# LukasHaas/PIGEON

Measured on AMD Instinct MI355X. Metric: images/sec end-to-end (ViT+head+refine), 4x336x336, higher is better.
Workload: dtype f16

## Files before the change

### include/pigeon_hip.h

```cpp
#ifndef PIGEON_HIP_H
#define PIGEON_HIP_H

#include <stddef.h>
#include <stdint.h>

#ifdef __cplusplus
extern "C" {
#endif

#define PG_OK            0
#define PG_EINVAL       -1
#define PG_ENOMEM       -2
#define PG_EHIP         -3
#define PG_ESTATE       -4

#define PG_DTYPE_F32     0
#define PG_DTYPE_BF16    1
#define PG_DTYPE_F16     2
#define PG_DTYPE_F64     3

#define PG_ABI_VERSION   7

const char* pg_last_error(void);
int pg_abi_version(void);
int pg_device_count(void);

typedef struct pg_vit pg_vit;

typedef struct pg_vit_cfg {
    int32_t layers;
    int32_t image_size;
    int32_t patch;
    int32_t hidden;
    int32_t heads;
    int32_t mlp;
    float   ln_eps;
    int32_t max_chunk;
    int32_t mma_dtype;
    int32_t precise;
} pg_vit_cfg;

int pg_vit_create(pg_vit** out, int device, const pg_vit_cfg* cfg);
int pg_vit_load_weight(pg_vit* h, const char* name, const void* data, int dtype,
                       const int64_t* shape, int ndim);
int pg_vit_finalize(pg_vit* h);
int pg_vit_workspace_bytes(const pg_vit* h, int n_images, size_t* bytes);
int pg_vit_forward(pg_vit* h, const void* pixels, int pix_dtype, int n_images, float* emb_out,
                   void* workspace, size_t workspace_bytes, void* stream);
int pg_vit_forward_hidden(pg_vit* h, const void* pixels, int pix_dtype, int n_images, float* emb_out,
                          float* hidden_out, void* workspace, size_t workspace_bytes, void* stream);
int pg_vit_precise_workspace_bytes(const pg_vit* h, int n_images, size_t* bytes);
int pg_vit_precise_plan(int n_images, int32_t out[8]);
int pg_vit_forward_precise(pg_vit* h, const void* pixels, int pix_dtype, int n_images, float* emb_out, float* hidden_out,
                           void* workspace, size_t workspace_bytes, void* stream);
int pg_vit_graph(pg_vit* h, int on, int64_t* replays, int64_t* captures);
int pg_vit_destroy(pg_vit* h);
int pg_vit_mma_dtype(const pg_vit* h);

int pg_fingerprint(const void* data, size_t bytes, uint64_t seed, uint64_t out[2], void* stream);
int pg_vit_fingerprint(const pg_vit* h, uint64_t out[2]);

#define PG_PROF_CLASSES 9
int pg_vit_profile_enable(pg_vit* h, int on);
int pg_vit_profile_read(pg_vit* h, int64_t* launches , double* ms );
int pg_vit_profile_reset(pg_vit* h);

int pg_tune_gemm_stagger(float fraction);
int pg_tune_gemm_tail_rows(int rows);
int pg_tune_gemm_tail_shape(int min_k, int min_n);
int pg_tune_gemm_raster(int gn);
int pg_tune_gemm_mid(int on);
int pg_gemm_plan(int variant, int epi, int M, int N, int K, int* kernel, int* rows_main, int* rest);
int pg_tune_exact_attention(int use_f32_mfma);
int pg_tune_exact_products(int n);
int pg_tune_exact_fusion(int on);
int pg_vit_saturation_check(pg_vit* h, int on);
int pg_vit_saturation_read(pg_vit* h, int64_t* count, int reset);
int pg_vit_range_alarm_read(pg_vit* h, int64_t* rows, int reset);

int pg_head_forward(const float* emb, int B, int P, const float* W, const float* bias,
                    const double* centroids, int C, int k, float* logits,
                    float* topk_val, int64_t* topk_idx, int64_t* argmax, double* pred_llh, void* stream);

int pg_head_margin(const float* logits, int B, int C, const float* emb, int P, const float* W, float* margin, float* sens,
                   int64_t* top2, void* stream);

int pg_head_certainty(const float* logits, int B, int C, const float* emb, int P, const float* W, const int64_t* topk_idx, int kx,
                      const float* beta, const float* wstats, float* tol, int32_t* code, float* margin, float* sens, void* stream);

int pg_aux_heads_forward(const float* emb, int B, int P, const float* W, const float* bias, int n_reg, int n_climate, int n_month,
                         const float* beta, float* preds, int64_t* cls, float* tol, int32_t* code, float* row_tol, void* stream);

typedef struct pg_bank {
    const float*   proto_emb;
    const int64_t* cell_off;
    const float*   proto_lnglat;
    const int32_t* proto_count;
    const int64_t* member_off;
    const int64_t* member_idx;
    const float*   train_emb;
    const float*   train_lnglat;
    int64_t num_cells;
    int64_t num_protos;
    int64_t num_train;
} pg_bank;

int pg_refine_forward(const pg_bank* bank, const float* q, int B, int P, const double* init_llh,
                      const int64_t* cand, const float* cand_prob, int k, int topk,
                      float temperature, double max_refine_km, float* scratch,
                      float* out_llh, int64_t* out_cell, int32_t* out_choice, void* stream);

int pg_refine_forward_ex(const pg_bank* bank, const float* q, int B, int P, const double* init_llh,
                         const int64_t* cand, const float* cand_prob, int k, int topk, int n_eval,
                         float temperature, double max_refine_km, float* scratch12,
                         float* out_llh, int64_t* out_cell, int32_t* out_choice, int32_t* out_refined, void* stream);

int pg_refine_certainty(const pg_bank* bank, const float* q, int B, int P, const int64_t* cand, const float* cand_prob, int k,
                        int topk, int n_eval, const float* scratch12, const float* W, int C, const float* beta,
                        const float* wstats, float temperature, const int32_t* refined, const int32_t* choice,
                        float* tol, int32_t* code, void* stream);

int pg_requeue_append(const float* head_tol, const float* refine_tol, const int32_t* refine_code, int B, float thr, int force_all,
                      int64_t dst_base, int64_t flushed, int64_t cap, int64_t* counters, int64_t* slot_dst, int32_t* row_slot,
                      uint8_t* certain, int32_t* cause, void* stream);
int pg_rows_to_slots(const void* src, int64_t row_bytes, const int32_t* row_slot, int B, void* dst, void* stream);
int pg_requeue_take(const int64_t* slot_dst, int64_t cap, int64_t head, int n_valid, int n_pad, int64_t* dst_out, void* stream);
int pg_scatter_rows(const void* src, int64_t row_bytes, const int64_t* dst_row, int n, void* dst, int64_t dst_rows,
                    int64_t remap_wb, int64_t remap_b, int64_t remap_off, void* stream);
int pg_head_wstats(const float* W, int C, const float* beta, float* out2, void* stream);

int pg_embedding_debias(float* emb, int64_t n, int dim, const float* bias, void* stream);

typedef struct pg_prep pg_prep;
int pg_prep_create(pg_prep** out, int device, int in_h, int in_w);
int pg_prep_destroy(pg_prep* h);
int pg_prep_geometry(const pg_prep* h, int32_t* out6);
int pg_prep_workspace_bytes(const pg_prep* h, int n_images, size_t* bytes);
int pg_prep_forward(pg_prep* h, const void* images_u8, int n_images, void* out, int out_dtype, void* workspace,
                    size_t workspace_bytes, void* stream);

#define PG_PREP_ITEM_BYTES 80
#define PG_PREP_RAGGED_MAX_IMAGES 65535
typedef struct pg_prep_item {
    uint64_t src_off;
    int32_t in_h, in_w;
    int32_t new_h, new_w, top, left;
    int32_t ksize_h, ksize_v;
    int32_t row0, nrows;
    int32_t tmp_row;
    uint32_t bounds_h_off, kk_h_off, bounds_v_off, kk_v_off;
    int32_t reserved[3];
} pg_prep_item;
int pg_prep_ragged_plan(int n, const int32_t* hw, pg_prep_item* items_out, size_t* packed_bytes, size_t* workspace_bytes);
typedef struct pg_prep_ragged pg_prep_ragged;
int pg_prep_ragged_create(pg_prep_ragged** out, int device);
int pg_prep_ragged_destroy(pg_prep_ragged* h);
int pg_prep_ragged_forward(pg_prep_ragged* h, const void* packed_dev, size_t packed_bytes, const pg_prep_item* items_host, int n,
                           void* out, int out_dtype, void* workspace, size_t workspace_bytes, void* stream);

#define PG_COMM_ID_BYTES 128
int pg_comm_unique_id(void* id_out );
int pg_comm_init_rank(void** comm, int nranks, const void* unique_id , int rank);
int pg_comm_count(void* comm, int* nranks);
int pg_allgather(void* comm, const void* send, void* recv, size_t bytes_per_rank, void* stream);
int pg_allgather_many(void* comm, int count, const void* const* send, void* const* recv, const size_t* bytes_per_rank,
                      void* stream);
int pg_comm_destroy(void* comm);
int pg_comm_rccl_version(void);

int pg_proto_build(const float* train_emb, int panels, int64_t num_train, const int64_t* member_off,
                   const int64_t* member_idx, int64_t num_protos, float* proto_emb, void* stream);
int pg_haversine_matrix(const void* x, int x_dtype, const double* y, int N, int M, double* out, void* stream);
int pg_haversine_pairs(const double* x, const void* y, int y_dtype, int64_t N, double* out, void* stream);
int pg_smooth_labels(const double* distances, int N, int M, double constant, double* out, void* stream);

int pg_haversine_blocks(const double* pts, const int64_t* cell_off, const int64_t* mat_off, int C, double zero_as, double* out,
                        void* stream);
int pg_optics_graph(const double* dist, const int64_t* cell_off, const int64_t* mat_off, int C, int min_samples, int64_t* ordering,
                    double* core, double* reach, int64_t* pred, void* stream);
int pg_optics_plan(int64_t n, int min_samples, int32_t out[4]);
int pg_tune_optics_lds_points(int max_points);

int pg_op_gemm16(int dtype, const void* A, int64_t lda, const void* W, const float* bias, void* out, int64_t ldc,
                 int M, int N, int K, int epi, float qscale, int qcols, const float* aux,
                 int variant, void* stream);
int pg_op_gemm16_ld(int dtype, const void* A, int64_t lda, const void* W, int64_t ldw, const float* bias, void* out,
                    int64_t ldc, int M, int N, int K, int epi, float qscale, int qcols, const float* aux,
                    int variant, void* stream);
int pg_op_rowstat_cast(const float* x, void* x16, int dtype, float* rowstat, int64_t rows, float eps, void* stream);
int pg_op_gemm16_resid_stat(int dtype, const void* A, int64_t lda, const void* W, int64_t ldw, const float* bias, float* X,
                            int64_t ldc, void* x16, int64_t ldx, float* statpart, int M, int N, int K, int variant, void* stream);
int pg_op_rowstat_finalize(const float* statpart, int slots, float* rowstat, int64_t rows, float eps, void* stream);
int pg_op_gemm16_ln(int dtype, const void* A, int64_t lda, const void* W, int64_t ldw, const float* bias, const float* colsum,
                    const float* rowstat, void* out, int64_t ldc, int M, int N, int K, int epi, float qscale, int qcols,
                    int variant, void* stream);
int pg_op_layernorm(const float* x, const float* gamma, const float* beta, void* y, int out_dtype,
                    int64_t rows, float eps, void* stream);
int pg_op_attention(int dtype, const void* qkv, void* out, int n_images, void* stream);
int pg_op_im2col(const void* pixels, int pix_dtype, void* out, int out_dtype, int n_images, void* stream);
int pg_op_token_mean(const float* x, float* out, int n_images, void* stream);
int pg_op_cast_f32(const float* x, void* y, int out_dtype, int64_t n, void* stream);
int pg_op_preln(float* x, const float* cls, const float* pos0, const float* gamma, const float* beta, int64_t rows, float eps,
                void* x16, int x16_dtype, float* rowstat, void* stream);
int pg_op_gemm16_parts(int dtype, const void* A, int64_t lda, const void* W, int64_t ldw, const float* bias, float* parts,
                       int M, int N, int Kp, int S, void* stream);
int pg_op_x3_split(const float* x, void* y3, int64_t rows, int cols, int gelu, void* stream);
int pg_op_x3_layernorm(const float* x, const float* gamma, const float* beta, void* y3, int64_t rows, float eps, void* stream);
int pg_op_attention_f32(const float* qkv, float* out, int n_images, void* stream);
int pg_op_attention_x3(const float* qkv, void* out3, int n_images, void* stream);
int pg_op_x3_im2col(const void* pixels, int pix_dtype, void* out3, int n_images, void* stream);
int pg_op_sum_parts(const float* parts, int S, int64_t part_elems, float* dst, int64_t n, int resid, void* stream);

#ifdef __cplusplus
}
#endif
#endif
```

### pigeon_amd/_lib.py

```python
from __future__ import annotations

import ctypes as C
import os

_HERE = os.path.dirname(os.path.abspath(__file__))
LIB_PATH = os.environ.get("PIGEON_HIP_LIB") or os.path.join(_HERE, "libpigeon_hip.so")

PG_DTYPE_F32, PG_DTYPE_BF16, PG_DTYPE_F16, PG_DTYPE_F64 = 0, 1, 2, 3
EPI_QKV, EPI_GELU, EPI_RESID, EPI_PATCH, EPI_F32, EPI_RESID_STAT, EPI_QKV_LN, EPI_GELU_LN, EPI_GELU_X3 = 0, 1, 2, 3, 4, 5, 6, 7, 8
PROF_CLASSES = ["gemm_qkv", "gemm_out", "gemm_fc1", "gemm_fc2", "gemm_patch", "attention", "layernorm",
                "im2col", "token_mean"]


class PigeonHipError(RuntimeError):
    pass


class VitCfg(C.Structure):
    _fields_ = [("layers", C.c_int32), ("image_size", C.c_int32), ("patch", C.c_int32), ("hidden", C.c_int32),
                ("heads", C.c_int32), ("mlp", C.c_int32), ("ln_eps", C.c_float), ("max_chunk", C.c_int32),
                ("mma_dtype", C.c_int32), ("precise", C.c_int32)]


class Bank(C.Structure):
    _fields_ = [("proto_emb", C.c_void_p), ("cell_off", C.c_void_p), ("proto_lnglat", C.c_void_p),
                ("proto_count", C.c_void_p), ("member_off", C.c_void_p), ("member_idx", C.c_void_p),
                ("train_emb", C.c_void_p), ("train_lnglat", C.c_void_p),
                ("num_cells", C.c_int64), ("num_protos", C.c_int64), ("num_train", C.c_int64)]


class PrepItem(C.Structure):
    _fields_ = [("src_off", C.c_uint64), ("in_h", C.c_int32), ("in_w", C.c_int32), ("new_h", C.c_int32), ("new_w", C.c_int32),
                ("top", C.c_int32), ("left", C.c_int32), ("ksize_h", C.c_int32), ("ksize_v", C.c_int32), ("row0", C.c_int32),
                ("nrows", C.c_int32), ("tmp_row", C.c_int32), ("bounds_h_off", C.c_uint32), ("kk_h_off", C.c_uint32),
                ("bounds_v_off", C.c_uint32), ("kk_v_off", C.c_uint32), ("reserved", C.c_int32 * 3)]


PREP_ITEM_BYTES = 80
assert C.sizeof(PrepItem) == PREP_ITEM_BYTES


_P, _I, _I64, _F, _D, _SZ = C.c_void_p, C.c_int, C.c_int64, C.c_float, C.c_double, C.c_size_t
SIGNATURES = {
    "pg_last_error": (C.c_char_p, []),
    "pg_abi_version": (_I, []),
    "pg_device_count": (_I, []),
    "pg_vit_create": (_I, [C.POINTER(_P), _I, C.POINTER(VitCfg)]),
    "pg_vit_load_weight": (_I, [_P, C.c_char_p, _P, _I, C.POINTER(_I64), _I]),
    "pg_vit_finalize": (_I, [_P]),
    "pg_vit_workspace_bytes": (_I, [_P, _I, C.POINTER(_SZ)]),
    "pg_vit_forward": (_I, [_P, _P, _I, _I, _P, _P, _SZ, _P]),
    "pg_vit_forward_hidden": (_I, [_P, _P, _I, _I, _P, _P, _P, _SZ, _P]),
    "pg_vit_precise_workspace_bytes": (_I, [_P, _I, C.POINTER(_SZ)]),
    "pg_vit_forward_precise": (_I, [_P, _P, _I, _I, _P, _P, _P, _SZ, _P]),
    "pg_vit_graph": (_I, [_P, _I, C.POINTER(_I64), C.POINTER(_I64)]),
    "pg_vit_destroy": (_I, [_P]),
    "pg_vit_mma_dtype": (_I, [_P]),
    "pg_fingerprint": (_I, [_P, _SZ, C.c_uint64, C.POINTER(C.c_uint64), _P]),
    "pg_vit_fingerprint": (_I, [_P, C.POINTER(C.c_uint64)]),
    "pg_vit_profile_enable": (_I, [_P, _I]),
    "pg_vit_profile_read": (_I, [_P, C.POINTER(_I64), C.POINTER(_D)]),
    "pg_vit_profile_reset": (_I, [_P]),
    "pg_tune_gemm_stagger": (_I, [_F]),
    "pg_tune_gemm_tail_rows": (_I, [_I]),
    "pg_tune_gemm_tail_shape": (_I, [_I, _I]),
    "pg_tune_gemm_raster": (_I, [_I]),
    "pg_tune_gemm_mid": (_I, [_I]),
    "pg_tune_exact_attention": (_I, [_I]),
    "pg_tune_exact_products": (_I, [_I]),
    "pg_tune_exact_fusion": (_I, [_I]),
    "pg_gemm_plan": (_I, [_I, _I, _I, _I, _I, _P, _P, _P]),
    "pg_vit_saturation_check": (_I, [_P, _I]),
    "pg_vit_saturation_read": (_I, [_P, C.POINTER(_I64), _I]),
    "pg_vit_range_alarm_read": (_I, [_P, C.POINTER(_I64), _I]),
    "pg_comm_unique_id": (_I, [_P]),
    "pg_comm_init_rank": (_I, [C.POINTER(_P), _I, _P, _I]),
    "pg_comm_count": (_I, [_P, C.POINTER(_I)]),
    "pg_allgather": (_I, [_P, _P, _P, _SZ, _P]),
    "pg_allgather_many": (_I, [_P, _I, C.POINTER(_P), C.POINTER(_P), C.POINTER(_SZ), _P]),
    "pg_comm_destroy": (_I, [_P]),
    "pg_comm_rccl_version": (_I, []),
    "pg_prep_create": (_I, [C.POINTER(_P), _I, _I, _I]),
    "pg_prep_destroy": (_I, [_P]),
    "pg_prep_geometry": (_I, [_P, C.POINTER(C.c_int32)]),
    "pg_prep_workspace_bytes": (_I, [_P, _I, C.POINTER(_SZ)]),
    "pg_prep_forward": (_I, [_P, _P, _I, _P, _I, _P, _SZ, _P]),
    "pg_prep_ragged_plan": (_I, [_I, C.POINTER(C.c_int32), C.POINTER(PrepItem), C.POINTER(_SZ), C.POINTER(_SZ)]),
    "pg_prep_ragged_create": (_I, [C.POINTER(_P), _I]),
    "pg_prep_ragged_destroy": (_I, [_P]),
    "pg_prep_ragged_forward": (_I, [_P, _P, _SZ, C.POINTER(PrepItem), _I, _P, _I, _P, _SZ, _P]),
    "pg_proto_build": (_I, [_P, _I, _I64, _P, _P, _I64, _P, _P]),
    "pg_haversine_matrix": (_I, [_P, _I, _P, _I, _I, _P, _P]),
    "pg_haversine_pairs": (_I, [_P, _P, _I, _I64, _P, _P]),
    "pg_smooth_labels": (_I, [_P, _I, _I, _D, _P, _P]),
    "pg_haversine_blocks": (_I, [_P, _P, _P, _I, _D, _P, _P]),
    "pg_optics_graph": (_I, [_P, _P, _P, _I, _I, _P, _P, _P, _P, _P]),
    "pg_optics_plan": (_I, [_I64, _I, C.POINTER(C.c_int32)]),
    "pg_tune_optics_lds_points": (_I, [_I]),
    "pg_head_forward": (_I, [_P, _I, _I, _P, _P, _P, _I, _I, _P, _P, _P, _P, _P, _P]),
    "pg_head_margin": (_I, [_P, _I, _I, _P, _I, _P, _P, _P, _P, _P]),
    "pg_head_certainty": (_I, [_P, _I, _I, _P, _I, _P, _P, _I, _P, _P, _P, _P, _P, _P, _P]),
    "pg_aux_heads_forward": (_I, [_P, _I, _I, _P, _P, _I, _I, _I, _P, _P, _P, _P, _P, _P, _P]),
    "pg_refine_forward": (_I, [C.POINTER(Bank), _P, _I, _I, _P, _P, _P, _I, _I, _F, _D, _P, _P, _P, _P, _P]),
    "pg_refine_forward_ex": (_I, [C.POINTER(Bank), _P, _I, _I, _P, _P, _P, _I, _I, _I, _F, _D, _P, _P, _P, _P, _P, _P]),
    "pg_refine_certainty": (_I, [C.POINTER(Bank), _P, _I, _I, _P, _P, _I, _I, _I, _P, _P, _I, _P, _P, _F, _P, _P, _P, _P, _P]),
    "pg_requeue_append": (_I, [_P, _P, _P, _I, _F, _I, _I64, _I64, _I64, _P, _P, _P, _P, _P, _P]),
    "pg_rows_to_slots": (_I, [_P, _I64, _P, _I, _P, _P]),
    "pg_requeue_take": (_I, [_P, _I64, _I64, _I, _I, _P, _P]),
    "pg_scatter_rows": (_I, [_P, _I64, _P, _I, _P, _I64, _I64, _I64, _I64, _P]),
    "pg_head_wstats": (_I, [_P, _I, _P, _P, _P]),
    "pg_embedding_debias": (_I, [_P, _I64, _I, _P, _P]),
    "pg_op_gemm16": (_I, [_I, _P, _I64, _P, _P, _P, _I64, _I, _I, _I, _I, _F, _I, _P, _I, _P]),
    "pg_op_gemm16_ld": (_I, [_I, _P, _I64, _P, _I64, _P, _P, _I64, _I, _I, _I, _I, _F, _I, _P, _I, _P]),
    "pg_op_rowstat_cast": (_I, [_P, _P, _I, _P, _I64, _F, _P]),
    "pg_op_gemm16_resid_stat": (_I, [_I, _P, _I64, _P, _I64, _P, _P, _I64, _P, _I64, _P, _I, _I, _I, _I, _P]),
    "pg_op_rowstat_finalize": (_I, [_P, _I, _P, _I64, _F, _P]),
    "pg_op_gemm16_ln": (_I, [_I, _P, _I64, _P, _I64, _P, _P, _P, _P, _I64, _I, _I, _I, _I, _F, _I, _I, _P]),
    "pg_op_layernorm": (_I, [_P, _P, _P, _P, _I, _I64, _F, _P]),
    "pg_op_attention": (_I, [_I, _P, _P, _I, _P]),
    "pg_op_im2col": (_I, [_P, _I, _P, _I, _I, _P]),
    "pg_op_token_mean": (_I, [_P, _P, _I, _P]),
    "pg_op_cast_f32": (_I, [_P, _P, _I, _I64, _P]),
    "pg_op_gemm16_parts": (_I, [_I, _P, _I64, _P, _I64, _P, _P, _I, _I, _I, _I, _P]),
    "pg_op_x3_split": (_I, [_P, _P, _I64, _I, _I, _P]),
    "pg_op_x3_layernorm": (_I, [_P, _P, _P, _P, _I64, _F, _P]),
    "pg_op_attention_f32": (_I, [_P, _P, _I, _P]),
    "pg_op_attention_x3": (_I, [_P, _P, _I, _P]),
    "pg_op_x3_im2col": (_I, [_P, _I, _P, _I, _P]),
    "pg_op_sum_parts": (_I, [_P, _I, _I64, _P, _I64, _I, _P]),
    "pg_op_preln": (_I, [_P, _P, _P, _P, _P, _I64, _F, _P, _I, _P, _P]),
    "pg_vit_precise_plan": (_I, [_I, C.POINTER(C.c_int32)]),
}

_lib = None


def load():
    global _lib
    if _lib is not None:
        return _lib
    if not os.path.exists(LIB_PATH):
        raise PigeonHipError(
            f"{LIB_PATH} not found: build it with `python -m pigeon_amd.build` (hipcc, gfx950). "
            "pigeon_amd has no CPU/PyTorch fallback for its hot path.")
    import torch
    lib = C.CDLL(LIB_PATH)
    for name, (res, args) in SIGNATURES.items():
        fn = getattr(lib, name)
        fn.restype = res
        fn.argtypes = args
    _lib = lib
    return lib


def check(rc: int, what: str = ""):
    if rc != 0:
        msg = load().pg_last_error()
        raise PigeonHipError(f"{what} failed (code {rc}): {msg.decode() if msg else ''}")


def require_gpu():
    lib = load()
    n = lib.pg_device_count()
    if n <= 0:
        raise PigeonHipError("pigeon_amd needs an AMD GPU (gfx950) visible to HIP; found none. "
                             "There is no CPU fallback for the hot path.")
    return n
```

### pigeon_amd/csrc/head.hip

```cpp
#include "common.h"
#include "pigeon_internal.h"
#include "certainty_common.h"
#include <cfloat>

#define HT 64
#define HK 32

__global__ __launch_bounds__(256) void head_logits_kernel(const float* __restrict__ emb, int B, int P,
                                                          const float* __restrict__ W, const float* __restrict__ bias,
                                                          int C, float* __restrict__ logits) {
    __shared__ float As[HK][HT + 1];
    __shared__ float Ws[HK][HT + 1];
    const int tid = threadIdx.x;
    const int c0 = blockIdx.x * HT, b0 = blockIdx.y * HT;
    const int tx = tid & 15, ty = tid >> 4;
    float acc[4][4];
#pragma unroll
    for (int i = 0; i < 4; ++i)
#pragma unroll
        for (int j = 0; j < 4; ++j) acc[i][j] = 0.f;
    const float invP = 1.0f / (float)P;
    for (int k0 = 0; k0 < VIT_HIDDEN; k0 += HK) {
#pragma unroll
        for (int i = 0; i < 8; ++i) {
            const int idx = tid + i * 256;
            const int r = idx >> 5, k = idx & 31;
            float a = 0.f;
            if (b0 + r < B) {
                const float* e = emb + ((int64_t)(b0 + r) * P) * VIT_HIDDEN + k0 + k;
                for (int p = 0; p < P; ++p) a += e[(int64_t)p * VIT_HIDDEN];
                a *= invP;
            }
            As[k][r] = a;
            Ws[k][r] = (c0 + r < C) ? W[(int64_t)(c0 + r) * VIT_HIDDEN + k0 + k] : 0.f;
        }
        __syncthreads();
#pragma unroll
        for (int k = 0; k < HK; ++k) {
            float a[4], w[4];
#pragma unroll
            for (int i = 0; i < 4; ++i) a[i] = As[k][ty * 4 + i];
#pragma unroll
            for (int j = 0; j < 4; ++j) w[j] = Ws[k][tx * 4 + j];
#pragma unroll
            for (int i = 0; i < 4; ++i)
#pragma unroll
                for (int j = 0; j < 4; ++j) acc[i][j] = fmaf(a[i], w[j], acc[i][j]);
        }
        __syncthreads();
    }
#pragma unroll
    for (int i = 0; i < 4; ++i) {
        const int b = b0 + ty * 4 + i;
        if (b >= B) continue;
#pragma unroll
        for (int j = 0; j < 4; ++j) {
            const int c = c0 + tx * 4 + j;
            if (c < C) logits[(int64_t)b * C + c] = acc[i][j] + bias[c];
        }
    }
}

struct ValIdx { float v; int i; };
__device__ __forceinline__ ValIdx block_argbest(ValIdx x, ValIdx* red ) {
#pragma unroll
    for (int o = 32; o >= 1; o >>= 1) {
        const float ov = __shfl_xor(x.v, o, 64);
        const int oi = __shfl_xor(x.i, o, 64);
        if (better(ov, oi, x.v, x.i)) { x.v = ov; x.i = oi; }
    }
    const int wave = threadIdx.x >> 6;
    __syncthreads();
    if ((threadIdx.x & 63) == 0) red[wave] = x;
    __syncthreads();
    ValIdx r = red[0];
#pragma unroll
    for (int w = 1; w < 4; ++w) if (better(red[w].v, red[w].i, r.v, r.i)) r = red[w];
    return r;
}

template <bool GLOBAL>
__global__ __launch_bounds__(256) void head_row_kernel(const float* __restrict__ logits, int C, int k,
                                                       const double* __restrict__ centroids,
                                                       float* __restrict__ topk_val, int64_t* __restrict__ topk_idx,
                                                       int64_t* __restrict__ argmax_out, double* __restrict__ pred_llh,
                                                       float* __restrict__ scratch) {
    extern __shared__ __attribute__((aligned(16))) float probs_lds[];
    float* probs = GLOBAL ? scratch + (int64_t)blockIdx.x * C : probs_lds;
    __shared__ ValIdx red[4];
    __shared__ float redf[4];
    const int b = blockIdx.x, tid = threadIdx.x;
    const float* row = logits + (int64_t)b * C;
    float mx = -FLT_MAX;
    for (int c = tid; c < C; c += 256) { const float v = row[c]; probs[c] = v; mx = fmaxf(mx, v); }
    mx = wave_max(mx);
    if ((tid & 63) == 0) redf[tid >> 6] = mx;
    __syncthreads();
    mx = fmaxf(fmaxf(redf[0], redf[1]), fmaxf(redf[2], redf[3]));
    __syncthreads();
    float sm = 0.f;
    for (int c = tid; c < C; c += 256) { const float e = expf(probs[c] - mx); probs[c] = e; sm += e; }
    sm = wave_sum(sm);
    if ((tid & 63) == 0) redf[tid >> 6] = sm;
    __syncthreads();
    sm = (redf[0] + redf[1]) + (redf[2] + redf[3]);
    for (int c = tid; c < C; c += 256) probs[c] = probs[c] / sm;
    __syncthreads();
    for (int r = 0; r < k; ++r) {
        ValIdx best; best.v = -1.f; best.i = 0x7fffffff;
        for (int c = tid; c < C; c += 256) {
            const float v = probs[c];
            if (better(v, c, best.v, best.i)) { best.v = v; best.i = c; }
        }
        best = block_argbest(best, red);
        if (tid == 0) {
            if (best.i < 0 || best.i >= C) best.i = r < C ? r : C - 1;
            topk_val[(int64_t)b * k + r] = best.v;
            topk_idx[(int64_t)b * k + r] = best.i;
            if (r == 0) {
                argmax_out[b] = best.i;
                pred_llh[2 * b] = centroids[2 * (int64_t)best.i];
                pred_llh[2 * b + 1] = centroids[2 * (int64_t)best.i + 1];
            }
            probs[best.i] = -2.f;
        }
        if (GLOBAL) __threadfence_block();
        __syncthreads();
    }
}

extern "C" int pg_head_forward(const float* emb, int B, int P, const float* W, const float* bias,
                               const double* centroids, int C, int k, float* logits, float* topk_val,
                               int64_t* topk_idx, int64_t* argmax, double* pred_llh, void* stream) {
    hipStream_t s = (hipStream_t)stream;
    if (B < 0) { pg_set_error("head: B = %d", B); return PG_EINVAL; }
    if (B == 0) return PG_OK;
    if (!emb || !W || !bias || !centroids || !logits || !topk_val || !topk_idx || !argmax || !pred_llh) {
        pg_set_error("head: null pointer argument"); return PG_EINVAL;
    }
    if (P < 1 || C < 1 || k < 1 || k > C) { pg_set_error("head: bad P=%d C=%d k=%d", P, C, k); return PG_EINVAL; }
    const size_t lds = (size_t)C * sizeof(float);
    const bool big = lds > 150 * 1024;
    dim3 g1((C + HT - 1) / HT, (B + HT - 1) / HT);
    hipLaunchKernelGGL(head_logits_kernel, g1, dim3(256), 0, s, emb, B, P, W, bias, C, logits);
    int rc = pg_check_launch("head_logits");
    if (rc) return rc;
    if (big) {
        float* scratch = nullptr;
        PG_HIP(hipMallocAsync((void**)&scratch, (size_t)B * C * sizeof(float), s));
        hipLaunchKernelGGL(head_row_kernel<true>, dim3(B), dim3(256), 0, s, logits, C, k, centroids, topk_val, topk_idx, argmax, pred_llh, scratch);
        rc = pg_check_launch("head_row (large C)");
        (void)hipFreeAsync(scratch, s);
        return rc;
    }
    static size_t attr_lds = 0;
    if (lds > attr_lds) {
        PG_HIP(hipFuncSetAttribute((const void*)head_row_kernel<false>, hipFuncAttributeMaxDynamicSharedMemorySize, (int)lds));
        attr_lds = lds;
    }
    hipLaunchKernelGGL(head_row_kernel<false>, dim3(B), dim3(256), lds, s, logits, C, k, centroids, topk_val, topk_idx, argmax, pred_llh,
                       (float*)nullptr);
    return pg_check_launch("head_row");
}

__global__ __launch_bounds__(256) void head_margin_kernel(const float* __restrict__ logits, int C, const float* __restrict__ emb, int P,
                                                          const float* __restrict__ W, float* __restrict__ margin,
                                                          float* __restrict__ sens, int64_t* __restrict__ top2) {
    __shared__ ValIdx red[4];
    __shared__ float redf[8];
    const int b = blockIdx.x, tid = threadIdx.x;
    const float* row = logits + (int64_t)b * C;
    ValIdx b1; b1.v = -FLT_MAX; b1.i = 0x7fffffff;
    bool any = false;
    for (int c = tid; c < C; c += 256) { const float v = row[c]; if (!any || better(v, c, b1.v, b1.i)) { b1.v = v; b1.i = c; any = true; } }
    if (!any) { b1.v = -FLT_MAX; b1.i = 0x7fffffff; }
    const ValIdx t1 = block_argbest(b1, red);
    ValIdx b2; b2.v = -FLT_MAX; b2.i = 0x7fffffff;
    any = false;
    for (int c = tid; c < C; c += 256) {
        if (c == t1.i) continue;
        const float v = row[c];
        if (!any || better(v, c, b2.v, b2.i)) { b2.v = v; b2.i = c; any = true; }
    }
    if (!any) { b2.v = -FLT_MAX; b2.i = 0x7fffffff; }
    __syncthreads();
    const ValIdx t2 = block_argbest(b2, red);
    const bool have2 = C > 1 && t2.i >= 0 && t2.i < C;
    float se = 0.f, sw = 0.f;
    {
        const int c0 = tid * 4;
        const float invP = 1.0f / (float)P;
#pragma unroll
        for (int e = 0; e < 4; ++e) {
            float a = 0.f;
            for (int p = 0; p < P; ++p) a += emb[((int64_t)b * P + p) * VIT_HIDDEN + c0 + e];
            a *= invP;
            se += a * a;
            if (have2) { const float d = W[(int64_t)t1.i * VIT_HIDDEN + c0 + e] - W[(int64_t)t2.i * VIT_HIDDEN + c0 + e]; sw += d * d; }
        }
    }
    se = wave_sum(se); sw = wave_sum(sw);
    __syncthreads();
    if ((tid & 63) == 0) { redf[tid >> 6] = se; redf[4 + (tid >> 6)] = sw; }
    __syncthreads();
    if (tid == 0) {
        se = (redf[0] + redf[1]) + (redf[2] + redf[3]);
        sw = (redf[4] + redf[5]) + (redf[6] + redf[7]);
        margin[b] = have2 ? t1.v - t2.v : INFINITY;
        sens[b] = have2 ? sqrtf(se) * sqrtf(sw) * (1.0f / 32.0f) : 0.f;
        if (top2) top2[b] = have2 ? t2.i : t1.i;
    }
}

extern "C" int pg_head_margin(const float* logits, int B, int C, const float* emb, int P, const float* W, float* margin, float* sens,
                              int64_t* top2, void* stream) {
    if (B < 0) { pg_set_error("head_margin: B = %d", B); return PG_EINVAL; }
    if (B == 0) return PG_OK;
    if (!logits || !emb || !W || !margin || !sens) { pg_set_error("head_margin: null pointer argument"); return PG_EINVAL; }
    if (P < 1 || C < 1) { pg_set_error("head_margin: bad P=%d C=%d", P, C); return PG_EINVAL; }
    hipLaunchKernelGGL(head_margin_kernel, dim3(B), dim3(256), 0, (hipStream_t)stream, logits, C, emb, P, W, margin, sens, top2);
    return pg_check_launch("head_margin");
}
```

### pigeon_amd/hip_ops.py

```python
from __future__ import annotations

import ctypes as C
from typing import Dict, Optional

import torch

from . import _lib
from ._lib import Bank, VitCfg, check, load

TOKENS, HIDDEN, MLP, PATCHES, KPAD = 577, 1024, 4096, 576, 640


def _p(t: Optional[torch.Tensor]):
    return C.c_void_p(0) if t is None else C.c_void_p(t.data_ptr())


def _stream():
    return C.c_void_p(torch.cuda.current_stream().cuda_stream)


_T16 = {torch.float16: _lib.PG_DTYPE_F16, torch.bfloat16: _lib.PG_DTYPE_BF16}
_PIXDT = {torch.float32: _lib.PG_DTYPE_F32, torch.float16: _lib.PG_DTYPE_F16, torch.bfloat16: _lib.PG_DTYPE_BF16}
_PG2T = {_lib.PG_DTYPE_F16: torch.float16, _lib.PG_DTYPE_BF16: torch.bfloat16, _lib.PG_DTYPE_F32: torch.float32}

# ... 671 lines not shown
    y = torch.empty((rows, 3 * cols), dtype=torch.float16, device=x.device)
    check(load().pg_op_x3_split(_p(x), _p(y), rows, cols, 1 if gelu else 0, _stream()), "pg_op_x3_split")
    return y


def gemm16_parts(A: torch.Tensor, W: torch.Tensor, bias: Optional[torch.Tensor], S: int) -> torch.Tensor:
    _dev(A); _dev(W)
    if W.dtype != A.dtype or A.shape[1] != W.shape[1] or A.shape[1] % S:
        raise _lib.PigeonHipError("gemm16_parts: A and W must share dtype and a K' divisible by S")
    M, Kt = A.shape
    N = W.shape[0]
    out = torch.empty((S, M, N), dtype=torch.float32, device=A.device)
    check(load().pg_op_gemm16_parts(_dt16(A), _p(A), A.stride(0), _p(W), W.stride(0), _p(bias), _p(out), M, N, Kt // S, S, _stream()),
          "pg_op_gemm16_parts")
    return out


def x3_layernorm(x: torch.Tensor, gamma: torch.Tensor, beta: torch.Tensor, eps: float = 1e-5) -> torch.Tensor:
    _dev(x, torch.float32)
    rows = x.numel() // HIDDEN
    y = torch.empty((rows, 3 * HIDDEN), dtype=torch.float16, device=x.device)
    check(load().pg_op_x3_layernorm(_p(x), _p(gamma), _p(beta), _p(y), rows, float(eps), _stream()), "pg_op_x3_layernorm")
    return y


def x3_pack_weight(W: torch.Tensor) -> torch.Tensor:
    Wh = W.to(torch.float16)
    Wl = ((W - Wh.float()) * 256.0).to(torch.float16)
    return torch.cat([Wh, Wh, Wl], dim=1).contiguous()


def attention_f32(qkv: torch.Tensor, n_images: int) -> torch.Tensor:
    _dev(qkv, torch.float32)
    _shape(qkv, "qkv", n_images * TOKENS, 3 * HIDDEN)
    out = torch.empty((n_images * TOKENS, HIDDEN), dtype=torch.float32, device=qkv.device)
    check(load().pg_op_attention_f32(_p(qkv), _p(out), n_images, _stream()), "pg_op_attention_f32")
    return out


class DeviceBank:

    FIELDS = [("proto_emb", torch.float32), ("cell_off", torch.int64), ("proto_lnglat", torch.float32),
              ("proto_count", torch.int32), ("member_off", torch.int64), ("member_idx", torch.int64),
              ("train_emb", torch.float32), ("train_lnglat", torch.float32)]

    def __init__(self, arrays, device="cuda"):
        self.t = {}
        for name, dt in self.FIELDS:
            a = getattr(arrays, name) if not isinstance(arrays, dict) else arrays[name]
            t = torch.as_tensor(a) if not torch.is_tensor(a) else a
            self.t[name] = t.to(device=device, dtype=dt).contiguous()
        self.num_cells = self.t["cell_off"].numel() - 1
        self.num_protos = self.t["proto_emb"].shape[0]
        self.num_train = self.t["train_emb"].shape[0]
        t = self.t
        _shape(t["proto_emb"], "proto_emb", self.num_protos, HIDDEN); _shape(t["proto_lnglat"], "proto_lnglat", self.num_protos, 2)
        _shape(t["proto_count"], "proto_count", self.num_protos); _shape(t["member_off"], "member_off", self.num_protos + 1)
        _shape(t["cell_off"], "cell_off", self.num_cells + 1); _shape(t["member_idx"], "member_idx", None)
        _shape(t["train_emb"], "train_emb", self.num_train, HIDDEN); _shape(t["train_lnglat"], "train_lnglat", self.num_train, 2)
        self.struct = Bank(*[C.c_void_p(self.t[n].data_ptr()) for n, _ in self.FIELDS],
                           self.num_cells, self.num_protos, self.num_train)


def refine_forward(bank: DeviceBank, q: torch.Tensor, init_llh: torch.Tensor, cand: torch.Tensor,
                   cand_prob: Optional[torch.Tensor], topk: int, temperature: float, max_refine_km: float,
                   return_scratch: bool = False):
    _dev(q, torch.float32); _dev(init_llh, torch.float64); _dev(cand, torch.int64)
    if cand_prob is not None:
        _dev(cand_prob, torch.float32)
    if q.dim() not in (2, 3) or cand.dim() != 2:
        raise _lib.PigeonHipError(f"refine: q must be (B,{HIDDEN}) or (B,P,{HIDDEN}) and cand (B,k), got {tuple(q.shape)} / {tuple(cand.shape)}")
    B = q.shape[0]
    P = q.shape[1] if q.dim() == 3 else 1
    k = cand.shape[1]
    _shape(q, "q", *((B, P, HIDDEN) if q.dim() == 3 else (B, HIDDEN)))
    _shape(init_llh, "init_llh", B, 2); _shape(cand, "cand", B, k)
    if cand_prob is not None:
        _shape(cand_prob, "cand_prob", B, k)
    if not 1 <= int(topk) <= k:
        raise _lib.PigeonHipError(f"refine: topk = {topk} of k = {k} candidates")
    dev = q.device
    scratch = torch.empty((B, topk, 4), dtype=torch.float32, device=dev)
    out_llh = torch.empty((B, 2), dtype=torch.float32, device=dev)
    out_cell = torch.empty((B,), dtype=torch.int64, device=dev)
    out_choice = torch.empty((B,), dtype=torch.int32, device=dev)
    check(load().pg_refine_forward(C.byref(bank.struct), _p(q), B, P, _p(init_llh), _p(cand), _p(cand_prob), k, topk,
                                   float(temperature), float(max_refine_km), _p(scratch), _p(out_llh), _p(out_cell),
                                   _p(out_choice), _stream()), "pg_refine_forward")
    if return_scratch:
        return out_llh, out_cell, out_choice, scratch
    return out_llh, out_cell, out_choice


def refine_forward_ex(bank: DeviceBank, q: torch.Tensor, init_llh: torch.Tensor, cand: torch.Tensor,
                      cand_prob: Optional[torch.Tensor], topk: int, n_eval: int, temperature: float, max_refine_km: float):
    _dev(q, torch.float32); _dev(init_llh, torch.float64); _dev(cand, torch.int64)
    if cand_prob is not None:
        _dev(cand_prob, torch.float32)
    if q.dim() not in (2, 3) or cand.dim() != 2:
        raise _lib.PigeonHipError(f"refine: q must be (B,{HIDDEN}) or (B,P,{HIDDEN}) and cand (B,k), got {tuple(q.shape)} / {tuple(cand.shape)}")
    B = q.shape[0]
    P = q.shape[1] if q.dim() == 3 else 1
    k = cand.shape[1]
    _shape(q, "q", *((B, P, HIDDEN) if q.dim() == 3 else (B, HIDDEN)))
    _shape(init_llh, "init_llh", B, 2); _shape(cand, "cand", B, k)
    if cand_prob is not None:
        _shape(cand_prob, "cand_prob", B, k)
    if not 1 <= int(topk) <= int(n_eval) <= k:
        raise _lib.PigeonHipError(f"refine_ex: topk = {topk}, n_eval = {n_eval} of k = {k} candidates")
    dev = q.device
    scratch = torch.empty((B, n_eval, 12), dtype=torch.float32, device=dev)
    out_llh = torch.empty((B, 2), dtype=torch.float32, device=dev)
    out_cell = torch.empty((B,), dtype=torch.int64, device=dev)
    out_choice = torch.empty((B,), dtype=torch.int32, device=dev)
    out_refined = torch.empty((B,), dtype=torch.int32, device=dev)
    check(load().pg_refine_forward_ex(C.byref(bank.struct), _p(q), B, P, _p(init_llh), _p(cand), _p(cand_prob), k, int(topk), int(n_eval),
                                      float(temperature), float(max_refine_km), _p(scratch), _p(out_llh), _p(out_cell),
                                      _p(out_choice), _p(out_refined), _stream()), "pg_refine_forward_ex")
    return out_llh, out_cell, out_choice, out_refined, scratch


def refine_certainty(bank: DeviceBank, q: torch.Tensor, cand: torch.Tensor, cand_prob: Optional[torch.Tensor], topk: int,
                     scratch12: torch.Tensor, W: torch.Tensor, drift: Optional[torch.Tensor], wstats: torch.Tensor,
                     temperature: float, refined: torch.Tensor, choice: torch.Tensor):
    _dev(q, torch.float32); _dev(cand, torch.int64); _dev(scratch12, torch.float32); _dev(W, torch.float32)
    _dev(wstats, torch.float32); _dev(refined, torch.int32); _dev(choice, torch.int32)
    B = q.shape[0]
    P = q.shape[1] if q.dim() == 3 else 1
    k = cand.shape[1]
    n_eval = scratch12.shape[1]
    _shape(q, "q", *((B, P, HIDDEN) if q.dim() == 3 else (B, HIDDEN)))
    _shape(cand, "cand", B, k); _shape(scratch12, "scratch12", B, n_eval, 12); _shape(W, "W", None, HIDDEN)
    _shape(refined, "refined", B); _shape(choice, "choice", B); _shape(wstats, "wstats", 2)
    if cand_prob is not None:
        _dev(cand_prob, torch.float32); _shape(cand_prob, "cand_prob", B, k)
    if drift is not None:
        _dev(drift, torch.float32); _shape(drift, "drift", HIDDEN)
    tol = torch.empty((B,), dtype=torch.float32, device=q.device)
    code = torch.empty((B,), dtype=torch.int32, device=q.device)
    check(load().pg_refine_certainty(C.byref(bank.struct), _p(q), B, P, _p(cand), _p(cand_prob), k, int(topk), int(n_eval), _p(scratch12),
                                     _p(W), W.shape[0], _p(drift), _p(wstats), float(temperature), _p(refined), _p(choice), _p(tol),
                                     _p(code), _stream()), "pg_refine_certainty")
    return tol, code


def tune_gemm_raster(gn: int) -> None:
    check(load().pg_tune_gemm_raster(int(gn)), "pg_tune_gemm_raster")


def tune_exact_fusion(on: bool) -> None:
    check(load().pg_tune_exact_fusion(1 if on else 0), "pg_tune_exact_fusion")


def tune_gemm_mid(on) -> None:
    mode = 2 if (not isinstance(on, bool) and on == 2) else (1 if on else 0)
    check(load().pg_tune_gemm_mid(mode), "pg_tune_gemm_mid")


def vit_precise_plan(n_images: int) -> dict:
    out = (C.c_int32 * 8)()
    check(load().pg_vit_precise_plan(int(n_images), out), "pg_vit_precise_plan")
    return dict(qkv=out[0], out=out[1], fc1=out[2], fc2=out[3], fc1_fused=bool(out[4]), attn_x3=bool(out[5]), chunk=out[6], chunks=out[7])


def tune_exact_products(n: int) -> None:
    check(load().pg_tune_exact_products(int(n)), "pg_tune_exact_products")


def x3_im2col(pixels: torch.Tensor, out: Optional[torch.Tensor] = None) -> torch.Tensor:
    _dev(pixels); _shape(pixels, "pixels", None, 3, 336, 336)
    n = pixels.shape[0]
    if out is None:
        out = torch.empty((n * PATCHES, 3 * KPAD), dtype=torch.float16, device=pixels.device)
    _dev(out, torch.float16)
    if out.numel() < n * PATCHES * 3 * KPAD:
        raise _lib.PigeonHipError("x3_im2col: output too small")
    check(load().pg_op_x3_im2col(_p(pixels), _PIXDT[pixels.dtype], _p(out), n, _stream()), "pg_op_x3_im2col")
    return out


def sum_parts(parts: torch.Tensor, dst: torch.Tensor, resid: bool, n: Optional[int] = None) -> torch.Tensor:
    _dev(parts, torch.float32); _dev(dst, torch.float32)
    S, pe = parts.shape[0], parts[0].numel()
    n = pe if n is None else int(n)
    if dst.numel() < n:
        raise _lib.PigeonHipError("sum_parts: dst too small")
    check(load().pg_op_sum_parts(_p(parts), S, pe, _p(dst), n, 1 if resid else 0, _stream()), "pg_op_sum_parts")
    return dst


def preln(x: torch.Tensor, cls: torch.Tensor, pos0: torch.Tensor, gamma: torch.Tensor, beta: torch.Tensor, rows: Optional[int] = None,
          eps: float = 1e-5, stat_dtype: Optional[torch.dtype] = None, x16: Optional[torch.Tensor] = None,
          rowstat: Optional[torch.Tensor] = None):
    _dev(x, torch.float32)
    for t in (cls, pos0, gamma, beta):
        _dev(t, torch.float32)
        if t.numel() < HIDDEN:
            raise _lib.PigeonHipError("preln: parameter vectors need 1024 elements")
    rows = x.numel() // HIDDEN if rows is None else int(rows)
    if x.numel() < rows * HIDDEN:
        raise _lib.PigeonHipError("preln: x too small")
    if stat_dtype is not None and x16 is None:
        x16 = torch.empty((rows, HIDDEN), dtype=stat_dtype, device=x.device)
        rowstat = torch.empty((rows, 2), dtype=torch.float32, device=x.device)
    if x16 is not None and (x16.numel() < rows * HIDDEN or rowstat.numel() < rows * 2):
        raise _lib.PigeonHipError("preln: x16 / rowstat too small")
    check(load().pg_op_preln(_p(x), _p(cls), _p(pos0), _p(gamma), _p(beta), rows, float(eps), _p(x16),
                             _dt16(x16) if x16 is not None else 0, _p(rowstat), _stream()), "pg_op_preln")
    return (x16, rowstat) if x16 is not None else None


def attention_x3(qkv: torch.Tensor, n_images: int, out: Optional[torch.Tensor] = None) -> torch.Tensor:
    _dev(qkv, torch.float32)
    _shape(qkv, "qkv", n_images * TOKENS, 3 * HIDDEN)
    if out is None:
        out = torch.empty((n_images * TOKENS, 3 * HIDDEN), dtype=torch.float16, device=qkv.device)
    _dev(out, torch.float16)
    if out.numel() < n_images * TOKENS * 3 * HIDDEN:
        raise _lib.PigeonHipError("attention_x3: output too small")
    check(load().pg_op_attention_x3(_p(qkv), _p(out), n_images, _stream()), "pg_op_attention_x3")
    return out
```

Measured before the change: 2463.

## Stream head weights through double-buffered LDS with DPP broadcast FMAs after separate mean

Replaces the head logits kernel with a two-step path. The patch mean is computed first into a scratch buffer, then a weight-streaming GEMV-style kernel runs. It double-buffers W column tiles through LDS, prefetches the next stage while computing, and uses inline-asm DPP row broadcast FMAs so each lane owns one class column and keeps small batches in registers. The goal is to make the head bandwidth-bound on W rather than recomputing the mean per tile, at the cost of an extra allocation and launch, and of fragile hand-written asm.

```diff
diff --git a/include/pigeon_hip.h b/include/pigeon_hip.h
--- a/include/pigeon_hip.h
+++ b/include/pigeon_hip.h
@@ -78,6 +78,7 @@
 int pg_vit_saturation_read(pg_vit* h, int64_t* count, int reset);
 int pg_vit_range_alarm_read(pg_vit* h, int64_t* rows, int reset);
 
+int pg_tune_head_stream(int on);
 int pg_head_forward(const float* emb, int B, int P, const float* W, const float* bias,
                     const double* centroids, int C, int k, float* logits,
                     float* topk_val, int64_t* topk_idx, int64_t* argmax, double* pred_llh, void* stream);
diff --git a/pigeon_amd/_lib.py b/pigeon_amd/_lib.py
--- a/pigeon_amd/_lib.py
+++ b/pigeon_amd/_lib.py
@@ -97,6 +97,7 @@
     "pg_optics_graph": (_I, [_P, _P, _P, _I, _I, _P, _P, _P, _P, _P]),
     "pg_optics_plan": (_I, [_I64, _I, C.POINTER(C.c_int32)]),
     "pg_tune_optics_lds_points": (_I, [_I]),
+    "pg_tune_head_stream": (_I, [_I]),
     "pg_head_forward": (_I, [_P, _I, _I, _P, _P, _P, _I, _I, _P, _P, _P, _P, _P, _P]),
     "pg_head_margin": (_I, [_P, _I, _I, _P, _I, _P, _P, _P, _P, _P]),
     "pg_head_certainty": (_I, [_P, _I, _I, _P, _I, _P, _P, _I, _P, _P, _P, _P, _P, _P, _P]),
diff --git a/pigeon_amd/csrc/head.hip b/pigeon_amd/csrc/head.hip
--- a/pigeon_amd/csrc/head.hip
+++ b/pigeon_amd/csrc/head.hip
@@ -59,6 +59,217 @@
             if (c < C) logits[(int64_t)b * C + c] = acc[i][j] + bias[c];
         }
     }
+}
+
+#define HS_CT 64
+
+__global__ __launch_bounds__(256) void head_panel_mean_kernel(const float* __restrict__ emb, int B, int P, float* __restrict__ mean) {
+    const int64_t i = (int64_t)blockIdx.x * 256 + threadIdx.x;
+    if (i >= (int64_t)B * VIT_HIDDEN) return;
+    const int64_t b = i / VIT_HIDDEN;
+    const int k = (int)(i % VIT_HIDDEN);
+    const float* e = emb + (b * P) * VIT_HIDDEN + k;
+    float a = 0.f;
+    for (int p = 0; p < P; ++p) a += e[(int64_t)p * VIT_HIDDEN];
+    a *= 1.0f / (float)P;
+    mean[i] = a;
+}
+
+#define HS_FM4(J, WOP)                                                                   \
+    "v_fmac_f32_dpp %0, %4, %" WOP " row_newbcast:" J " row_mask:0xf bank_mask:0xf\n\t"    \
+    "v_fmac_f32_dpp %1, %5, %" WOP " row_newbcast:" J " row_mask:0xf bank_mask:0xf\n\t"    \
+    "v_fmac_f32_dpp %2, %6, %" WOP " row_newbcast:" J " row_mask:0xf bank_mask:0xf\n\t"    \
+    "v_fmac_f32_dpp %3, %7, %" WOP " row_newbcast:" J " row_mask:0xf bank_mask:0xf\n\t"
+#define HS_FM2(J, WOP)                                                                   \
+    "v_fmac_f32_dpp %0, %2, %" WOP " row_newbcast:" J " row_mask:0xf bank_mask:0xf\n\t"    \
+    "v_fmac_f32_dpp %1, %3, %" WOP " row_newbcast:" J " row_mask:0xf bank_mask:0xf\n\t"
+#define HS_W16(w) "v"(w[0]), "v"(w[1]), "v"(w[2]), "v"(w[3]), "v"(w[4]), "v"(w[5]), "v"(w[6]), "v"(w[7]), \
+                  "v"(w[8]), "v"(w[9]), "v"(w[10]), "v"(w[11]), "v"(w[12]), "v"(w[13]), "v"(w[14]), "v"(w[15])
+
+__device__ __forceinline__ void hs_fma16x4(float* acc, const float* a, const float (&w)[16]) {
+    asm("s_nop 4\n\t"
+        HS_FM4("0", "8") HS_FM4("1", "9") HS_FM4("2", "10") HS_FM4("3", "11")
+        HS_FM4("4", "12") HS_FM4("5", "13") HS_FM4("6", "14") HS_FM4("7", "15")
+        HS_FM4("8", "16") HS_FM4("9", "17") HS_FM4("10", "18") HS_FM4("11", "19")
+        HS_FM4("12", "20") HS_FM4("13", "21") HS_FM4("14", "22") HS_FM4("15", "23")
+        : "+v"(acc[0]), "+v"(acc[1]), "+v"(acc[2]), "+v"(acc[3])
+        : "v"(a[0]), "v"(a[1]), "v"(a[2]), "v"(a[3]), HS_W16(w));
+}
+__device__ __forceinline__ void hs_fma16x2(float* acc, const float* a, const float (&w)[16]) {
+    asm("s_nop 4\n\t"
+        HS_FM2("0", "4") HS_FM2("1", "5") HS_FM2("2", "6") HS_FM2("3", "7")
+        HS_FM2("4", "8") HS_FM2("5", "9") HS_FM2("6", "10") HS_FM2("7", "11")
+        HS_FM2("8", "12") HS_FM2("9", "13") HS_FM2("10", "14") HS_FM2("11", "15")
+        HS_FM2("12", "16") HS_FM2("13", "17") HS_FM2("14", "18") HS_FM2("15", "19")
+        : "+v"(acc[0]), "+v"(acc[1])
+        : "v"(a[0]), "v"(a[1]), HS_W16(w));
+}
+
+template <int KC, int NB>
+__device__ __forceinline__ void hs_stage(float (&acc)[NB], const float (&a)[KC / 16][NB], const float* cur, const int lane) {
+    static_assert(NB == 2 || NB % 4 == 0, "rows per wave");
+#pragma unroll
+    for (int sub = 0; sub < KC / 16; ++sub) {
+        float w[16];
+#pragma unroll
+        for (int q = 0; q < 4; ++q) {
+            const float4 v = *reinterpret_cast<const float4*>(&cur[lane * (KC + 4) + sub * 16 + q * 4]);
+            w[q * 4] = v.x; w[q * 4 + 1] = v.y; w[q * 4 + 2] = v.z; w[q * 4 + 3] = v.w;
+        }
+        if constexpr (NB == 2) {
+            hs_fma16x2(&acc[0], &a[sub][0], w);
+        } else {
+#pragma unroll
+            for (int r0 = 0; r0 < NB; r0 += 4) hs_fma16x4(&acc[r0], &a[sub][r0], w);
+        }
+    }
+}
+
+template <int KC, int NB>
+__global__ __launch_bounds__(256, KC == 64 ? 3 : 2) void head_logits_stream_kernel(const float* __restrict__ mean, int B,
+                                                                                   const float* __restrict__ W,
+                                                                                   const float* __restrict__ bias, int C,
+                                                                                   float* __restrict__ logits, int row_blocks) {
+    constexpr int LD = KC + 4;
+    constexpr int NS = VIT_HIDDEN / KC;
+    constexpr int TPR = KC / 4;
+    constexpr int RPP = 256 / TPR;
+    constexpr int NLD = HS_CT / RPP;
+    constexpr int NSUB = KC / 16;
+    static_assert(NS % 2 == 0 && NS >= 4, "the stage loop is unrolled by two");
+    extern __shared__ __attribute__((aligned(16))) float hs_w[];
+    const int tid = threadIdx.x, lane = tid & 63, wave = tid >> 6;
+    int tile = blockIdx.x, rblk = 0;
+    if (row_blocks > 1) {
+        const int slot = blockIdx.x >> 3;
+        tile = (slot / row_blocks) * 8 + (blockIdx.x & 7);
+        rblk = slot % row_blocks;
+    }
+    const int c0 = tile * HS_CT;
+    if (c0 >= C) return;
+    const int b0 = (rblk * 4 + wave) * NB;
+
+    const int scol = (tid % TPR) * 4, srow = tid / TPR;
+    const char* wbase = reinterpret_cast<const char*>(W + (int64_t)c0 * VIT_HIDDEN);
+    const int clast = C - 1 - c0;
+    unsigned woff[NLD];
+#pragma unroll
+    for (int i = 0; i < NLD; ++i) {
+        int c = srow + i * RPP;
+        c = c < clast ? c : clast;
+        woff[i] = (unsigned)(c * VIT_HIDDEN + scol) * 4u;
+    }
+    const int bblk = rblk * 4 * NB;
+    const char* abase = reinterpret_cast<const char*>(mean + (int64_t)bblk * VIT_HIDDEN);
+    const int blast = B - 1 - bblk;
+    unsigned aoff[NB];
+#pragma unroll
+    for (int r = 0; r < NB; ++r) {
+        int b = wave * NB + r;
+        b = b < blast ? b : blast;
+        aoff[r] = (unsigned)(b * VIT_HIDDEN + (lane & 15)) * 4u;
+    }
+    auto ld_w = [&](const int i, const int k) { return *reinterpret_cast<const float4*>(wbase + ((size_t)woff[i] + (size_t)k * 4)); };
+    auto ld_a = [&](const int r, const int k) { return *reinterpret_cast<const float*>(abase + ((size_t)aoff[r] + (size_t)k * 4)); };
+    float acc[NB];
+#pragma unroll
+    for (int r = 0; r < NB; ++r) acc[r] = 0.f;
+
+    float a0[NSUB][NB], a1[NSUB][NB];
+#pragma unroll
+    for (int sub = 0; sub < NSUB; ++sub)
+#pragma unroll
+        for (int r = 0; r < NB; ++r) a0[sub][r] = ld_a(r, sub * 16);
+    {
+        float4 stg[NLD];
+#pragma unroll
+        for (int i = 0; i < NLD; ++i) stg[i] = ld_w(i, 0);
+#pragma unroll
+        for (int i = 0; i < NLD; ++i) *reinterpret_cast<float4*>(&hs_w[(srow + i * RPP) * LD + scol]) = stg[i];
+    }
+    __syncthreads();
+    auto step = [&](const int s, const float (&au)[NSUB][NB], float (&al)[NSUB][NB]) __attribute__((always_inline)) {
+        const float* cur = hs_w + (s & 1) * (HS_CT * LD);
+        float* nxt = hs_w + ((s + 1) & 1) * (HS_CT * LD);
+        float4 stg[NLD];
+#pragma unroll
+        for (int sub = 0; sub < NSUB; ++sub)
+#pragma unroll
+            for (int r = 0; r < NB; ++r) al[sub][r] = ld_a(r, (s + 1) * KC + sub * 16);
+#pragma unroll
+        for (int i = 0; i < NLD; ++i) stg[i] = ld_w(i, (s + 1) * KC);
+        __builtin_amdgcn_sched_barrier(0);
+        hs_stage<KC, NB>(acc, au, cur, lane);
+#pragma unroll
+        for (int i = 0; i < NLD; ++i) *reinterpret_cast<float4*>(&nxt[(srow + i * RPP) * LD + scol]) = stg[i];
+        __syncthreads();
+    };
+    for (int s = 0; s + 2 < NS; s += 2) {
+        step(s, a0, a1);
+        step(s + 1, a1, a0);
+    }
+    step(NS - 2, a0, a1);
+    hs_stage<KC, NB>(acc, a1, hs_w + ((NS - 1) & 1) * (HS_CT * LD), lane);
+    const int c = c0 + lane;
+    if (c >= C) return;
+    const float bc = bias[c];
+#pragma unroll
+    for (int r = 0; r < NB; ++r) {
+        const int b = b0 + r;
+        if (b < B) logits[(int64_t)b * C + c] = acc[r] + bc;
+    }
+}
+
+static int g_head_stream = -1;
+extern "C" int pg_tune_head_stream(int on) {
+    g_head_stream = on ? 1 : 0;
+    return PG_OK;
+}
+static bool head_stream_on() {
+    if (g_head_stream < 0) { const char* e = getenv("PIGEON_HEAD_STREAM"); g_head_stream = (e && e[0] == '0') ? 0 : 1; }
+    return g_head_stream != 0;
+}
+
+static int head_logits_stream_launch(const float* emb, int B, int P, const float* W, const float* bias, int C, float* logits,
+                                     hipStream_t s) {
+    float* mean = nullptr;
+    PG_HIP(hipMallocAsync((void**)&mean, (size_t)B * VIT_HIDDEN * sizeof(float), s));
+    const int64_t n = (int64_t)B * VIT_HIDDEN;
+    hipLaunchKernelGGL(head_panel_mean_kernel, dim3((unsigned)((n + 255) / 256)), dim3(256), 0, s, emb, B, P, mean);
+    int rc = pg_check_launch("head_panel_mean");
+    if (!rc) {
+        const unsigned gx = (unsigned)((C + HS_CT - 1) / HS_CT);
+        constexpr int lds128 = 2 * HS_CT * (128 + 4) * (int)sizeof(float);
+        constexpr int lds64 = 2 * HS_CT * (64 + 4) * (int)sizeof(float);
+        if (B <= 32) {
+            static bool attr_set = false;
+            if (!attr_set) {
+                hipError_t e = hipFuncSetAttribute((const void*)head_logits_stream_kernel<128, 2>, hipFuncAttributeMaxDynamicSharedMemorySize, lds128);
+                if (e == hipSuccess)
+                    e = hipFuncSetAttribute((const void*)head_logits_stream_kernel<128, 8>, hipFuncAttributeMaxDynamicSharedMemorySize, lds128);
+                if (e != hipSuccess) {
+                    pg_set_error("head: %d bytes of LDS: %s", lds128, hipGetErrorString(e));
+                    (void)hipFreeAsync(mean, s);
+                    return PG_EHIP;
+                }
+                attr_set = true;
+            }
+            if (B <= 8) hipLaunchKernelGGL((head_logits_stream_kernel<128, 2>), dim3(gx), dim3(256), lds128, s, mean, B, W, bias, C, logits, 1);
+            else hipLaunchKernelGGL((head_logits_stream_kernel<128, 8>), dim3(gx), dim3(256), lds128, s, mean, B, W, bias, C, logits, 1);
+        } else {
+            const int rb = (B + 31) / 32;
+            if ((int64_t)((gx + 7) / 8) * 8 * rb > 0x7fffffffLL) {
+                pg_set_error("head: B = %d x C = %d is more blocks than a launch takes", B, C);
+                (void)hipFreeAsync(mean, s);
+                return PG_EINVAL;
+            }
+            hipLaunchKernelGGL((head_logits_stream_kernel<64, 8>), dim3((gx + 7) / 8 * 8 * (unsigned)rb), dim3(256), lds64, s, mean, B, W, bias, C,
+                               logits, rb);
+        }
+        rc = pg_check_launch("head_logits_stream");
+    }
+    (void)hipFreeAsync(mean, s);
+    return rc;
 }
 
 struct ValIdx { float v; int i; };
@@ -141,9 +352,14 @@
     if (P < 1 || C < 1 || k < 1 || k > C) { pg_set_error("head: bad P=%d C=%d k=%d", P, C, k); return PG_EINVAL; }
     const size_t lds = (size_t)C * sizeof(float);
     const bool big = lds > 150 * 1024;
-    dim3 g1((C + HT - 1) / HT, (B + HT - 1) / HT);
-    hipLaunchKernelGGL(head_logits_kernel, g1, dim3(256), 0, s, emb, B, P, W, bias, C, logits);
-    int rc = pg_check_launch("head_logits");
+    int rc;
+    if (head_stream_on() && ((uintptr_t)W & 15) == 0) {
+        rc = head_logits_stream_launch(emb, B, P, W, bias, C, logits, s);
+    } else {
+        dim3 g1((C + HT - 1) / HT, (B + HT - 1) / HT);
+        hipLaunchKernelGGL(head_logits_kernel, g1, dim3(256), 0, s, emb, B, P, W, bias, C, logits);
+        rc = pg_check_launch("head_logits");
+    }
     if (rc) return rc;
     if (big) {
         float* scratch = nullptr;
diff --git a/pigeon_amd/hip_ops.py b/pigeon_amd/hip_ops.py
--- a/pigeon_amd/hip_ops.py
+++ b/pigeon_amd/hip_ops.py
@@ -847,6 +847,10 @@
     check(load().pg_tune_exact_fusion(1 if on else 0), "pg_tune_exact_fusion")
 
 
+def tune_head_stream(on: bool) -> None:
+    check(load().pg_tune_head_stream(1 if on else 0), "pg_tune_head_stream")
+
+
 def tune_gemm_mid(on) -> None:
     mode = 2 if (not isinstance(on, bool) and on == 2) else (1 if on else 0)
     check(load().pg_tune_gemm_mid(mode), "pg_tune_gemm_mid")
```

Result: no change. 2469 (median of 6 runs) (+0.2%).
